# eltoto1219/vltk

Hardware: AMD Instinct MI355X
Metric: images/sec FRCNN feature extraction, 800x1333 batch (higher is better)
Workload: dtype f16

## Files before the change

vltk_amd/csrc/conv_ws.hip:

```cpp
#include "vk_common.h"

#include <cstdio>
#include <type_traits>
#include <vector>

namespace vk {

typedef _Float16 half8 __attribute__((ext_vector_type(8)));
typedef float floatx4 __attribute__((ext_vector_type(4)));
typedef _Float16 half4 __attribute__((ext_vector_type(4)));
typedef unsigned uintx4 __attribute__((ext_vector_type(4)));
typedef _Float16 half2v __attribute__((ext_vector_type(2)));

struct WsK {
    const char *x;
    const char *x2;
    const char *w;
    const float *bias;
    const char *res;
    char *y;
    int M;
    int kbytes;
    int ldy;
    int relu;
    int m_tiles, n_tiles;
    unsigned long *stamps;
    double *pool;
    int HW;
    int H, W, Wo, HoWo, stride;
};

#define VKW_GLDS16(gptr, lptr)                                                                         \
    __builtin_amdgcn_global_load_lds((const __attribute__((address_space(1))) void *)(gptr),          \
                                     (__attribute__((address_space(3))) void *)(lptr), 16, 0, 0)

template <int N>
__device__ __forceinline__ void ws_vm_wait() {
    asm volatile("s_waitcnt vmcnt(%0)" ::"n"(N) : "memory");
}

constexpr int WS_BM = 64;

template <int KC, int NW, int DBG = 0, bool POOL = false, bool DUAL = false, bool STRIDED = false>
__global__ __launch_bounds__(NW * 64, 1) void conv_ws_kernel(WsK p) {
    extern __shared__ __attribute__((aligned(16))) char smem[];
    static_assert(!DUAL || KC == 4, "two sources: 64 + 64 channels");
    constexpr int SCH = KC == 2 ? 64 : 128;
    constexpr int KSL = SCH / 32;
    constexpr int PITCH = SCH * 2;
    constexpr int WS_SLOT = WS_BM * PITCH;
    constexpr int WS_NS = 6;
    constexpr int WS_D = 5;
    constexpr int RING = WS_NS * WS_SLOT;
    constexpr int SPT = KC / KSL;
    constexpr int NI = 16 / NW;
    constexpr int WCH = NI * 16;
    constexpr int PPW = WS_SLOT / 1024 / NW;
    constexpr int RPW = 32 / NW;
    constexpr int NU = NI * 2;
    static_assert(!POOL || NW == 8, "the fused-mean epilogue is written for 32 channels per wave");

    const int tid = threadIdx.x, lane = tid & 63;
    const int wave = __builtin_amdgcn_readfirstlane(tid >> 6);
    const int g = lane >> 4, j = lane & 15;

    const int wg = blockIdx.x, per_xcd = gridDim.x >> 3;
    const int xcd = wg & 7, i = wg >> 3;
    const int n_tile = i % p.n_tiles, lane_m = i / p.n_tiles;
    const int lanes_x = per_xcd / p.n_tiles;
    const int ML = 8 * lanes_x;
    const int first = xcd * lanes_x + lane_m;
    const int ntw = first < p.m_tiles ? (p.m_tiles - first + ML - 1) / ML : 0;
    const int n0 = n_tile * 256;
    const int total = ntw * SPT;

    half8 wf[NI][KC];
#pragma unroll
    for (int ni = 0; ni < NI; ++ni) {
        const int co = n0 + wave * WCH + (ni >> 1) * 32 + (j >> 2) * 8 + (ni & 1) * 4 + (j & 3);
        const char *wr = p.w + (long)co * (DUAL ? 256 : p.kbytes) + g * 16;
#pragma unroll
        for (int ks = 0; ks < KC; ++ks) wf[ni][ks] = *reinterpret_cast<const half8 *>(wr + ks * 64);
    }
    char *res_lds = smem + RING + wave * (WS_BM * WCH * 2);
    float *bias_lds = reinterpret_cast<float *>(smem + RING + 4 * WS_BM * 128);
    if (tid < 256) bias_lds[tid] = p.bias[n0 + tid];
    ws_vm_wait<0>();
    __syncthreads();

    constexpr int LPR = PITCH / 16;
    const int drow = lane / LPR, dslot = lane & (LPR - 1);
    auto request = [&](int q_, int qlo = 0, int qhi = WS_BM * (KC == 2 ? 128 : 256) / 1024 / NW) {
        const int it = q_ / SPT, st = q_ - it * SPT;
        const int m0 = (first + it * ML) * WS_BM;
        char *dst = smem + (q_ % WS_NS) * WS_SLOT + wave * PPW * 1024;
#pragma unroll
        for (int q = qlo; q < qhi; ++q) {
            const int row = (wave * PPW + q) * (64 / LPR) + drow;
            const int m = min(m0 + row, p.M - 1);
            if constexpr (STRIDED) {
                const int n_ = m / p.HoWo, r_ = m - n_ * p.HoWo;
                const int ho = r_ / p.Wo, wo = r_ - ho * p.Wo;
                const long src = ((long)n_ * p.H + ho * p.stride) * p.W + wo * p.stride;
                VKW_GLDS16(p.x + src * p.kbytes + st * PITCH + ((dslot ^ (row & (LPR - 1))) << 4), dst + q * 1024);
            } else if constexpr (DUAL) {
                const int c = dslot ^ (row & (LPR - 1));
                VKW_GLDS16((c < 8 ? p.x : p.x2) + (long)m * 128 + ((c & 7) << 4), dst + q * 1024);
            } else {
                VKW_GLDS16(p.x + (long)m * p.kbytes + st * PITCH + ((dslot ^ (row & (LPR - 1))) << 4), dst + q * 1024);
            }
        }
    };
    for (int q_ = 0; q_ < WS_D && q_ < total; ++q_) request(q_);

    int xoff[KSL];
#pragma unroll
    for (int ksl = 0; ksl < KSL; ++ksl) xoff[ksl] = j * PITCH + (((ksl * 4 + g) ^ (j & (LPR - 1))) << 4);

    unsigned long c_vm4[4] = {0, 0, 0, 0}, c_bar4[4] = {0, 0, 0, 0};
    unsigned long c_vm = 0, c_bar = 0, c_mma = 0, c_rw = 0, c_epi = 0, c_all = 0, t_a = 0, t_b = 0;
    if constexpr (DBG & 32) c_all = __builtin_amdgcn_s_memtime();
    floatx4 acc[4][NI];
    auto rsw = [](int r) { return (0x1320 >> (((r >> 2) & 3) * 4)) & 3; };
    auto epilogue = [&](int it_, auto res_c, auto relu_c, auto full_c) {
        constexpr bool RES = decltype(res_c)::value, RELU = decltype(relu_c)::value, FULL = decltype(full_c)::value;
        const long mbase = (long)(first + it_ * ML) * WS_BM;
        const long img0 = POOL ? mbase / p.HW : 0;
        const long m_split = (img0 + 1) * (POOL ? p.HW : 1);
        const bool two_images = POOL && m_split < mbase + WS_BM && m_split < p.M;
        unsigned *scr = reinterpret_cast<unsigned *>(res_lds);
        int ln = lane;
        if constexpr (POOL) asm volatile("" : "+v"(ln));
        const int gp = ln >> 4, jp = ln & 15;
#pragma unroll
        for (int u0 = 0; u0 < NU; u0 += 4) {
            half8 rr[4];
            if constexpr (RES) {
#pragma unroll
                for (int u = u0; u < u0 + 4; ++u) {
                    const int qn = u >> 2, row = (u & 3) * 16 + j;
                    if constexpr (NW == 4)
                        rr[u - u0] = *reinterpret_cast<const half8 *>(res_lds + row * 128 + (((qn * 4 + g) ^ (row & 7)) << 4));
                    else
                        rr[u - u0] = *reinterpret_cast<const half8 *>(res_lds + row * 64 + ((g ^ rsw(row)) << 4));
                }
            }
#pragma unroll
            for (int u = u0; u < u0 + 4; ++u) {
                const int qn = u >> 2, pt = u & 3;
                const int ch = wave * WCH + qn * 32 + g * 8;
                const floatx4 b0 = *reinterpret_cast<const floatx4 *>(bias_lds + ch), b1 = *reinterpret_cast<const floatx4 *>(bias_lds + ch + 4);
                floatx4 x0 = acc[pt][2 * qn] + b0, x1 = acc[pt][2 * qn + 1] + b1;
                if constexpr (RES) {
                    x0 += __builtin_convertvector(__builtin_shufflevector(rr[u - u0], rr[u - u0], 0, 1, 2, 3), floatx4);
                    x1 += __builtin_convertvector(__builtin_shufflevector(rr[u - u0], rr[u - u0], 4, 5, 6, 7), floatx4);
                }
                half4 h0 = __builtin_convertvector(x0, half4), h1 = __builtin_convertvector(x1, half4);
                half8 o = __builtin_shufflevector(h0, h1, 0, 1, 2, 3, 4, 5, 6, 7);
                if constexpr (RELU) o = __builtin_elementwise_max(o, half8{0, 0, 0, 0, 0, 0, 0, 0});
                const long m = mbase + pt * 16 + j;
                if constexpr (POOL) {
                    if (!FULL && m >= p.M) o = half8{0, 0, 0, 0, 0, 0, 0, 0};
                    const uintx4 ov = __builtin_bit_cast(uintx4, o);
#pragma unroll
                    for (int k = 0; k < 4; ++k) scr[(gp * 4 + k) * 64 + ((pt * 16 + jp + gp * 16) & 63)] = ov[k];
                } else {
                    if constexpr (DBG & 64) {
                        asm volatile("" ::"v"(o));
                    } else {
                        if (FULL || m < p.M) *reinterpret_cast<half8 *>(p.y + (m * p.ldy + n0 + ch) * 2) = o;
                    }
                }
            }
        }
        if constexpr (POOL) {
            const int pr = jp, q = gp;
            const uintx4 *src = reinterpret_cast<const uintx4 *>(scr + pr * 64 + ((q + (pr >> 2)) & 3) * 16);
            uintx4 v[4];
#pragma unroll
            for (int c4 = 0; c4 < 4; ++c4) v[c4] = src[c4];
            double a0 = 0.0, a1 = 0.0, b0 = 0.0, b1 = 0.0;
            if (!two_images) {
#pragma unroll
                for (int r = 0; r < 16; ++r) {
                    const unsigned d = v[r >> 2][r & 3];
                    const half2v h = __builtin_bit_cast(half2v, d);
                    a0 += (double)(float)h[0];
                    a1 += (double)(float)h[1];
                }
            } else {
                const int sloc = (int)(m_split - mbase);
#pragma unroll
                for (int r = 0; r < 16; ++r) {
                    const unsigned d = v[r >> 2][r & 3];
                    const half2v h = __builtin_bit_cast(half2v, d);
                    const bool second = q * 16 + r >= sloc;
                    const float lo = (float)h[0], hi = (float)h[1];
                    a0 += (double)(second ? 0.f : lo);
                    a1 += (double)(second ? 0.f : hi);
                    b0 += (double)(second ? lo : 0.f);
                    b1 += (double)(second ? hi : 0.f);
                }
            }
            a0 += __shfl_xor(a0, 16);
            a1 += __shfl_xor(a1, 16);
            a0 += __shfl_xor(a0, 32);
            a1 += __shfl_xor(a1, 32);
            double *dst = p.pool + img0 * p.ldy + n0 + wave * WCH + pr * 2;
            if (ln < 16) {
                unsafeAtomicAdd(dst, a0);
                unsafeAtomicAdd(dst + 1, a1);
            }
            if (two_images) {
                b0 += __shfl_xor(b0, 16);
                b1 += __shfl_xor(b1, 16);
                b0 += __shfl_xor(b0, 32);
                b1 += __shfl_xor(b1, 32);
                if (ln < 16) {
                    unsafeAtomicAdd(dst + p.ldy, b0);
                    unsafeAtomicAdd(dst + p.ldy + 1, b1);
                }
            }
        }
    };
    for (int it = 0; it < ntw; ++it) {
#pragma unroll
        for (int pt = 0; pt < 4; ++pt)
#pragma unroll
            for (int ni = 0; ni < NI; ++ni) acc[pt][ni] = floatx4{0.f, 0.f, 0.f, 0.f};
        const int m0 = (first + it * ML) * WS_BM;
        if (p.res && !(DBG & 8)) {
#pragma unroll
            for (int q = 0; q < RPW; ++q) {
                if constexpr (NW == 4) {
                    const int row = q * 8 + (lane >> 3);
                    const int m = min(m0 + row, p.M - 1);
                    VKW_GLDS16(p.res + ((long)m * p.ldy + n0 + wave * 64) * 2 + (((lane & 7) ^ (row & 7)) << 4), res_lds + q * 1024);
                } else {
                    const int row = q * 16 + (lane >> 2);
                    const int m = min(m0 + row, p.M - 1);
                    VKW_GLDS16(p.res + ((long)m * p.ldy + n0 + wave * 32) * 2 + (((lane & 3) ^ rsw(row)) << 4), res_lds + q * 1024);
                }
            }
        }
#pragma unroll
        for (int st = 0; st < SPT; ++st) {
            const int gs = it * SPT + st;
            if constexpr (DBG & 32) t_a = __builtin_amdgcn_s_memtime();
            if (gs + WS_D - 1 < total)
                ws_vm_wait<PPW * (WS_D - 1)>();
            else
                ws_vm_wait<0>();
            if constexpr (DBG & 32) {
                t_b = __builtin_amdgcn_s_memtime();
                c_vm += t_b - t_a;
                c_vm4[st & 3] += t_b - t_a;
            }
            __builtin_amdgcn_s_barrier();
            if constexpr (DBG & 32) {
                t_a = __builtin_amdgcn_s_memtime();
                c_bar += t_a - t_b;
                c_bar4[st & 3] += t_a - t_b;
            }
            const bool more = gs + WS_D < total && !(DBG & 4);
            const char *slot = smem + (gs % WS_NS) * WS_SLOT;
            half8 xf[KSL][4];
#pragma unroll
            for (int ksl = 0; ksl < KSL; ++ksl)
#pragma unroll
                for (int pt = 0; pt < 4; ++pt) xf[ksl][pt] = *reinterpret_cast<const half8 *>(slot + pt * 16 * PITCH + xoff[ksl]);
            __builtin_amdgcn_sched_barrier(0);
#pragma unroll
            for (int ksl = 0; ksl < KSL; ++ksl) {
#pragma unroll
                for (int pt = 0; pt < 4; ++pt)
#pragma unroll
                    for (int ni = 0; ni < NI; ++ni) {
                        if constexpr (DBG & 2) {
                            asm volatile("" ::"v"(xf[ksl][pt]));
                            continue;
                        }
                        acc[pt][ni] = __builtin_amdgcn_mfma_f32_16x16x32_f16(wf[ni][KSL * st + ksl], xf[ksl][pt], acc[pt][ni], 0, 0, 0);
                    }
                __builtin_amdgcn_sched_barrier(0);
                if constexpr (NW == 4) {
                    if (more) request(gs + WS_D, ksl, ksl + 1);
                } else {
                    if (more && (ksl & 1)) request(gs + WS_D, ksl >> 1, (ksl >> 1) + 1);
                }
                __builtin_amdgcn_sched_barrier(0);
            }
            if constexpr (DBG & 32) c_mma += __builtin_amdgcn_s_memtime() - t_a;
        }
        if constexpr (DBG & 32) t_a = __builtin_amdgcn_s_memtime();
        if constexpr (DBG & 1) {
#pragma unroll
            for (int pt = 0; pt < 4; ++pt)
#pragma unroll
                for (int ni = 0; ni < NI; ++ni) asm volatile("" ::"v"(acc[pt][ni]));
        }
        if (!(DBG & 1)) {
            if (p.res) {
                if ((it + 1) * SPT - 1 + WS_D < total)
                    ws_vm_wait<PPW * SPT>();
                else
                    ws_vm_wait<0>();
            }
            if constexpr (DBG & 32) {
                t_b = __builtin_amdgcn_s_memtime();
                c_rw += t_b - t_a;
            }
            const bool full = (long)(first + it * ML + 1) * WS_BM <= p.M;
            auto by_full = [&](auto r, auto l) {
                if (full)
                    epilogue(it, r, l, std::true_type{});
                else
                    epilogue(it, r, l, std::false_type{});
            };
            auto by_relu = [&](auto r) {
                if (p.relu)
                    by_full(r, std::true_type{});
                else
                    by_full(r, std::false_type{});
            };
            if (p.res)
                by_relu(std::true_type{});
            else
                by_relu(std::false_type{});
            if constexpr (DBG & 32) c_epi += __builtin_amdgcn_s_memtime() - t_b;
        }
    }
    if constexpr (DBG & 32) {
        if (lane == 0) {
            unsigned long *o = p.stamps + ((long)blockIdx.x * NW + wave) * 16;
            o[0] = __builtin_amdgcn_s_memtime() - c_all;
            o[1] = c_vm;
            o[2] = c_bar;
            o[3] = c_mma;
            o[4] = c_rw;
            o[5] = c_epi;
            o[6] = ntw;
            o[7] = __builtin_amdgcn_s_memrealtime();
            for (int q = 0; q < 4; ++q) {
                o[8 + q] = c_vm4[q];
                o[12 + q] = c_bar4[q];
            }
        }
    }
}

bool conv_pool_sums_f64(long N, int HW, int Cin, int Cout, bool dual) {
    const char *v = getenv("VK_CONV_WS");
    if (v && v[0] == '0') return false;
    const char *q = getenv("VK_WS_POOL");
    if (q && q[0] == '0') return false;
    if (dual || Cin != 512 || Cout % 256 != 0 || 32 % (Cout / 256) != 0) return false;
    const long M = N * HW;
    return HW >= 128 && HW <= 8192 && M >= 8 * 128 && M < (1L << 31) - 128;
}

bool conv_ws_pool_ok(const ConvArgs &a) {
    return a.pool_part && conv_duo_pool_ok(a) && a.relu <= 1 && a.ldy == a.Cout &&
           conv_pool_sums_f64(a.N, a.Ho * a.Wo, a.Cin, a.Cout, a.x2 != nullptr);
}

bool conv_ws_eligible(const ConvArgs &a) {
    const char *v = getenv("VK_CONV_WS");
    if (v && v[0] == '0') return false;
    if (a.pool_part) return conv_ws_pool_ok(a);
    if (a.stem || a.groups > 1 || a.dt != VK_F16 || a.out_dt != VK_F16 || a.relu > 1) return false;
    if (a.kh != 1 || a.kw != 1 || a.pad != 0 || a.stride < 1) return false;
    if (a.stride != 1) {
        const char *sv = getenv("VK_WS_STRIDED");
        if ((sv && sv[0] == '0') || a.x2 || a.res || (a.Cin != 256 && a.Cin != 512)) return false;
    }
    if (a.x2 && (a.Cin != 64 || a.Cin2 != 64)) return false;
    if (a.Cout % 256 != 0 || a.ldy != a.Cout || (a.Cin != 64 && a.Cin != 128 && a.Cin != 256 && a.Cin != 512)) return false;
    const int nt = a.Cout / 256;
    if (32 % nt != 0) return false;
    const long M = (long)a.N * a.Ho * a.Wo;
    return M >= 8 * 128 && M < (1L << 31) - 128;
}

template <int KC, int NW = 8, int DBG = 0, bool POOL = false, bool DUAL = false, bool STRIDED = false>
static int launch_ws(const WsK &k, hipStream_t stream) {
    constexpr int smem = 6 * WS_BM * 256 + 4 * WS_BM * 128 + 1024;
    VK_TRY(set_max_lds(conv_ws_kernel<KC, NW, DBG, POOL, DUAL, STRIDED>, smem));
    hipLaunchKernelGGL((conv_ws_kernel<KC, NW, DBG, POOL, DUAL, STRIDED>), dim3(256), dim3(NW * 64), smem, stream, k);
    VK_CHECK_HIP(hipGetLastError());
    return VK_OK;
}

int launch_conv_ws(const ConvArgs &a, hipStream_t stream) {
    WsK k;
    k.x = (const char *)a.x;
    k.x2 = (const char *)a.x2;
    k.w = (const char *)a.w;
    k.bias = a.bias;
    k.res = (const char *)a.res;
    k.y = (char *)a.y;
    const long M = (long)a.N * a.Ho * a.Wo;
    k.M = (int)M;
    k.kbytes = a.Cin * 2;
    k.ldy = a.ldy;
    k.relu = a.relu;
    k.m_tiles = (int)((M + WS_BM - 1) / WS_BM);
    k.n_tiles = a.Cout / 256;
    k.stamps = nullptr;
    k.pool = (double *)a.pool_part;
    k.HW = a.Ho * a.Wo;
    k.H = a.H;
    k.W = a.W;
    k.Wo = a.Wo;
    k.HoWo = a.Ho * a.Wo;
    k.stride = a.stride;

    Timed t;
    VK_TRY(t.begin(stream));
    int st;
    if (a.pool_part) {
        VK_CHECK_HIP(hipMemsetAsync(k.pool, 0, (size_t)(M / k.HW) * a.Cout * sizeof(double), stream));
        VK_TRY((launch_ws<16, 8, 0, true>(k, stream)));
        return t.end(stream, a.concurrent ? 6 : 8, 2.0 * (double)M * a.Cout * a.Cin, (int)M, a.Cout, a.Cin, 1, 1,
                     2.0 * ((double)M * a.Cin + (double)M * a.Cout * (a.res ? 1 : 0) + (double)a.Cout * a.Cin));
    }
    const char *nwv = getenv("VK_WS_WAVES");
    const int nw = nwv ? atoi(nwv) : 8;
#ifdef VK_ABLATION
    if (const char *sf = getenv("VK_WS_STAMPS")) {
        if (a.Cin != 512) return VK_EINVAL;
        const size_t nb = (size_t)256 * 8 * 16 * sizeof(unsigned long);
        VK_CHECK_HIP(hipMalloc((void **)&k.stamps, nb));
        VK_CHECK_HIP(hipMemsetAsync(k.stamps, 0, nb, stream));
        st = nw == 8 ? launch_ws<16, 8, 32>(k, stream) : launch_ws<16, 4, 32>(k, stream);
        VK_CHECK_HIP(hipStreamSynchronize(stream));
        std::vector<unsigned long> h(256 * 8 * 16);
        VK_CHECK_HIP(hipMemcpy(h.data(), k.stamps, nb, hipMemcpyDeviceToHost));
        VK_CHECK_HIP(hipFree(k.stamps));
        if (FILE *f = fopen(sf, "a")) {
            fprintf(f, "# wg wave total vm_wait barrier stage_body res_wait epilogue tiles realtime\n");
            for (int w = 0; w < 256 * nw; ++w) {
                fprintf(f, "%d %d", w / nw, w % nw);
                for (int i = 0; i < 16; ++i) fprintf(f, " %lu", h[(size_t)w * 16 + i]);
                fprintf(f, "\n");
            }
            fclose(f);
        }
    } else
#endif
    {
#ifdef VK_ABLATION
        const char *d = getenv("VK_WS_DBG");
        const int dbg = d ? atoi(d) : 0;
#define VKW_DBG_CASE(NW_, D_) \
    case D_: st = launch_ws<16, NW_, D_>(k, stream); break;
#else
        const int dbg = 0;
#define VKW_DBG_CASE(NW_, D_)
#endif
        if (a.stride != 1)
            st = a.Cin == 256 ? launch_ws<8, 8, 0, false, false, true>(k, stream) : launch_ws<16, 8, 0, false, false, true>(k, stream);
        else if (a.x2)
            st = launch_ws<4, 8, 0, false, true>(k, stream);
        else if (a.Cin == 64)
            st = nw == 8 ? launch_ws<2, 8>(k, stream) : launch_ws<2, 4>(k, stream);
        else if (a.Cin == 128)
            st = nw == 8 ? launch_ws<4, 8>(k, stream) : launch_ws<4, 4>(k, stream);
        else if (a.Cin == 256)
            st = nw == 8 ? launch_ws<8, 8>(k, stream) : launch_ws<8, 4>(k, stream);
        else if (nw == 8) {
            switch (dbg) {
                VKW_DBG_CASE(8, 1) VKW_DBG_CASE(8, 2) VKW_DBG_CASE(8, 3) VKW_DBG_CASE(8, 4) VKW_DBG_CASE(8, 8) VKW_DBG_CASE(8, 12)
                VKW_DBG_CASE(8, 15) VKW_DBG_CASE(8, 64) VKW_DBG_CASE(8, 9) VKW_DBG_CASE(8, 72)
                default: st = launch_ws<16, 8>(k, stream); break;
            }
        } else {
            switch (dbg) {
                VKW_DBG_CASE(4, 1) VKW_DBG_CASE(4, 2) VKW_DBG_CASE(4, 3) VKW_DBG_CASE(4, 4) VKW_DBG_CASE(4, 8) VKW_DBG_CASE(4, 12)
                VKW_DBG_CASE(4, 15)
                default: st = launch_ws<16, 4>(k, stream); break;
            }
        }
#undef VKW_DBG_CASE
    }
    VK_TRY(st);
    const int K = a.Cin + (a.x2 ? a.Cin2 : 0);
    return t.end(stream, a.concurrent ? 6 : 8, 2.0 * (double)M * a.Cout * K, (int)M, a.Cout, K, 1, 1,
                 2.0 * ((double)M * K + (double)M * a.Cout * (a.res ? 2 : 1) + (double)a.Cout * K));
}

}
```

Measured before the change: 483.5.

## Stage residual and output through whole-row LDS tiles for 512-channel conv

Adds a ROWS variant of the warp-specialized 1x1 conv kernel for 512-input-channel layers. It loads the residual tile as contiguous 512-byte rows with swizzled global-to-LDS loads issued during the first K stage, and writes outputs to LDS so they can be stored back as full coalesced rows after a barrier. The aim is to replace scattered 16-byte residual reads and output writes with wide contiguous transfers, and to hide the residual fetch behind the MFMA work. In exchange it adds a block-wide barrier per tile and changes the vmcnt wait accounting on the last stage, which could cause stalls or be fragile.

Result: no change. 484.9 (median of 6 runs) (+0.3%).

```diff
diff --git a/vltk_amd/csrc/conv_ws.hip b/vltk_amd/csrc/conv_ws.hip
--- a/vltk_amd/csrc/conv_ws.hip
+++ b/vltk_amd/csrc/conv_ws.hip
@@ -41,7 +41,7 @@
 
 constexpr int WS_BM = 64;
 
-template <int KC, int NW, int DBG = 0, bool POOL = false, bool DUAL = false, bool STRIDED = false>
+template <int KC, int NW, int DBG = 0, bool POOL = false, bool DUAL = false, bool STRIDED = false, bool ROWS = false>
 __global__ __launch_bounds__(NW * 64, 1) void conv_ws_kernel(WsK p) {
     extern __shared__ __attribute__((aligned(16))) char smem[];
     static_assert(!DUAL || KC == 4, "two sources: 64 + 64 channels");
@@ -59,6 +59,8 @@
     constexpr int RPW = 32 / NW;
     constexpr int NU = NI * 2;
     static_assert(!POOL || NW == 8, "the fused-mean epilogue is written for 32 channels per wave");
+    static_assert(!ROWS || (NW == 8 && SCH == 128 && SPT >= 2 && DBG == 0 && !POOL && !DUAL && !STRIDED),
+                  "whole-row residual / output: eight waves, 128-channel stages, a stage before the last one to request it in");
 
     const int tid = threadIdx.x, lane = tid & 63;
     const int wave = __builtin_amdgcn_readfirstlane(tid >> 6);
@@ -83,6 +85,7 @@
         for (int ks = 0; ks < KC; ++ks) wf[ni][ks] = *reinterpret_cast<const half8 *>(wr + ks * 64);
     }
     char *res_lds = smem + RING + wave * (WS_BM * WCH * 2);
+    char *img = smem + RING;
     float *bias_lds = reinterpret_cast<float *>(smem + RING + 4 * WS_BM * 128);
     if (tid < 256) bias_lds[tid] = p.bias[n0 + tid];
     ws_vm_wait<0>();
@@ -139,7 +142,9 @@
 #pragma unroll
                 for (int u = u0; u < u0 + 4; ++u) {
                     const int qn = u >> 2, row = (u & 3) * 16 + j;
-                    if constexpr (NW == 4)
+                    if constexpr (ROWS)
+                        rr[u - u0] = *reinterpret_cast<const half8 *>(img + row * 512 + (((wave * 4 + g) ^ (row & 15)) << 4));
+                    else if constexpr (NW == 4)
                         rr[u - u0] = *reinterpret_cast<const half8 *>(res_lds + row * 128 + (((qn * 4 + g) ^ (row & 7)) << 4));
                     else
                         rr[u - u0] = *reinterpret_cast<const half8 *>(res_lds + row * 64 + ((g ^ rsw(row)) << 4));
@@ -164,6 +169,9 @@
                     const uintx4 ov = __builtin_bit_cast(uintx4, o);
 #pragma unroll
                     for (int k = 0; k < 4; ++k) scr[(gp * 4 + k) * 64 + ((pt * 16 + jp + gp * 16) & 63)] = ov[k];
+                } else if constexpr (ROWS) {
+                    const int row = pt * 16 + j;
+                    *reinterpret_cast<half8 *>(img + row * 512 + (((wave * 4 + g) ^ (row & 15)) << 4)) = o;
                 } else {
                     if constexpr (DBG & 64) {
                         asm volatile("" ::"v"(o));
@@ -171,6 +179,22 @@
                         if (FULL || m < p.M) *reinterpret_cast<half8 *>(p.y + (m * p.ldy + n0 + ch) * 2) = o;
                     }
                 }
+            }
+        }
+        if constexpr (ROWS) {
+            asm volatile("s_waitcnt lgkmcnt(0)\n\ts_barrier" ::: "memory");
+            int ln = lane;
+            asm volatile("" : "+v"(ln));
+            half8 sv[4];
+#pragma unroll
+            for (int k = 0; k < 4; ++k) {
+                const int row = wave * 8 + k * 2 + (ln >> 5), c = ln & 31;
+                sv[k] = *reinterpret_cast<const half8 *>(img + row * 512 + ((c ^ (row & 15)) << 4));
+            }
+#pragma unroll
+            for (int k = 0; k < 4; ++k) {
+                const long m = mbase + wave * 8 + k * 2 + (ln >> 5);
+                if (FULL || m < p.M) *reinterpret_cast<half8 *>(p.y + (m * p.ldy + n0 + (ln & 31) * 8) * 2) = sv[k];
             }
         }
         if constexpr (POOL) {
@@ -229,7 +253,7 @@
 #pragma unroll
             for (int ni = 0; ni < NI; ++ni) acc[pt][ni] = floatx4{0.f, 0.f, 0.f, 0.f};
         const int m0 = (first + it * ML) * WS_BM;
-        if (p.res && !(DBG & 8)) {
+        if (p.res && !(DBG & 8) && !ROWS) {
 #pragma unroll
             for (int q = 0; q < RPW; ++q) {
                 if constexpr (NW == 4) {
@@ -247,10 +271,14 @@
         for (int st = 0; st < SPT; ++st) {
             const int gs = it * SPT + st;
             if constexpr (DBG & 32) t_a = __builtin_amdgcn_s_memtime();
-            if (gs + WS_D - 1 < total)
-                ws_vm_wait<PPW * (WS_D - 1)>();
-            else
+            if (gs + WS_D - 1 < total) {
+                if (ROWS && st == SPT - 1 && p.res)
+                    ws_vm_wait<ROWS ? PPW * (SPT - 1) - 1 : 0>();
+                else
+                    ws_vm_wait<PPW * (WS_D - 1)>();
+            } else {
                 ws_vm_wait<0>();
+            }
             if constexpr (DBG & 32) {
                 t_b = __builtin_amdgcn_s_memtime();
                 c_vm += t_b - t_a;
@@ -283,6 +311,18 @@
                         acc[pt][ni] = __builtin_amdgcn_mfma_f32_16x16x32_f16(wf[ni][KSL * st + ksl], xf[ksl][pt], acc[pt][ni], 0, 0, 0);
                     }
                 __builtin_amdgcn_sched_barrier(0);
+                if constexpr (ROWS) {
+                    if (st == 0 && p.res && !(ksl & 1)) {
+                        int ln = lane;
+                        asm volatile("" : "+v"(ln));
+#pragma unroll
+                        for (int q = (ksl >> 1) * 2; q < (ksl >> 1) * 2 + 2; ++q) {
+                            const int row = (wave * 4 + q) * 2 + (ln >> 5), c = (ln & 31) ^ (row & 15);
+                            const int m = min(m0 + row, p.M - 1);
+                            VKW_GLDS16(p.res + ((long)m * p.ldy + n0 + c * 8) * 2, img + (wave * 4 + q) * 1024);
+                        }
+                    }
+                }
                 if constexpr (NW == 4) {
                     if (more) request(gs + WS_D, ksl, ksl + 1);
                 } else {
@@ -300,7 +340,7 @@
                 for (int ni = 0; ni < NI; ++ni) asm volatile("" ::"v"(acc[pt][ni]));
         }
         if (!(DBG & 1)) {
-            if (p.res) {
+            if (p.res && !ROWS) {
                 if ((it + 1) * SPT - 1 + WS_D < total)
                     ws_vm_wait<PPW * SPT>();
                 else
@@ -382,11 +422,11 @@
     return M >= 8 * 128 && M < (1L << 31) - 128;
 }
 
-template <int KC, int NW = 8, int DBG = 0, bool POOL = false, bool DUAL = false, bool STRIDED = false>
+template <int KC, int NW = 8, int DBG = 0, bool POOL = false, bool DUAL = false, bool STRIDED = false, bool ROWS = false>
 static int launch_ws(const WsK &k, hipStream_t stream) {
     constexpr int smem = 6 * WS_BM * 256 + 4 * WS_BM * 128 + 1024;
-    VK_TRY(set_max_lds(conv_ws_kernel<KC, NW, DBG, POOL, DUAL, STRIDED>, smem));
-    hipLaunchKernelGGL((conv_ws_kernel<KC, NW, DBG, POOL, DUAL, STRIDED>), dim3(256), dim3(NW * 64), smem, stream, k);
+    VK_TRY(set_max_lds(conv_ws_kernel<KC, NW, DBG, POOL, DUAL, STRIDED, ROWS>, smem));
+    hipLaunchKernelGGL((conv_ws_kernel<KC, NW, DBG, POOL, DUAL, STRIDED, ROWS>), dim3(256), dim3(NW * 64), smem, stream, k);
     VK_CHECK_HIP(hipGetLastError());
     return VK_OK;
 }
@@ -426,6 +466,8 @@
     }
     const char *nwv = getenv("VK_WS_WAVES");
     const int nw = nwv ? atoi(nwv) : 8;
+    const char *rv = getenv("VK_WS_ROWS");
+    const bool rows = !(rv && rv[0] == '0');
 #ifdef VK_ABLATION
     if (const char *sf = getenv("VK_WS_STAMPS")) {
         if (a.Cin != 512) return VK_EINVAL;
@@ -472,7 +514,7 @@
             switch (dbg) {
                 VKW_DBG_CASE(8, 1) VKW_DBG_CASE(8, 2) VKW_DBG_CASE(8, 3) VKW_DBG_CASE(8, 4) VKW_DBG_CASE(8, 8) VKW_DBG_CASE(8, 12)
                 VKW_DBG_CASE(8, 15) VKW_DBG_CASE(8, 64) VKW_DBG_CASE(8, 9) VKW_DBG_CASE(8, 72)
-                default: st = launch_ws<16, 8>(k, stream); break;
+                default: st = rows ? launch_ws<16, 8, 0, false, false, false, true>(k, stream) : launch_ws<16, 8>(k, stream); break;
             }
         } else {
             switch (dbg) {
```
